# alanqrwang/nwhead

Measured on AMD Instinct MI355X. Metric: query-predictions/sec, higher is better.
Workload: dtype f32; 1 GPU; K3 predict('full'): B=256 queries/step vs bank N=50000 d=512 C=200, bank sharded 1-way, 26 query batches coalesced per launch; B=256, N_support=50000, d=512, C=200, parallelism=support-shard x1

## Files before the change

### nwhead_amd/csrc/fused.hip

```cpp
#include <mutex>
#include <utility>
#include <vector>
#include "fused_impl.h"
#include <cstring>

namespace nw {

#define NW_EXTERN_FUSED_KIND(K)                                                                          \
    extern template int launch_fused_kind<K>(const float*, const float*, const int64_t*, const float*,   \
                                             const float*,                                               \
                                             const float*, float*, float*, float*, float*, float*,       \
                                             float*, void*, size_t, int, int, int, int, hipStream_t);
NW_EXTERN_FUSED_KIND(NW_SCORE_EUCLIDEAN)
NW_EXTERN_FUSED_KIND(NW_SCORE_HYPERSPHERE)
NW_EXTERN_FUSED_KIND(NW_SCORE_COSINE)
NW_EXTERN_FUSED_KIND(NW_SCORE_DOT)
NW_EXTERN_FUSED_KIND(NW_SCORE_CLIP)
#undef NW_EXTERN_FUSED_KIND

namespace {
struct TileTimer {
    bool on = false;
    std::vector<std::pair<hipEvent_t, hipEvent_t>> ev;
    std::vector<std::pair<hipEvent_t, hipEvent_t>> pool;
    std::mutex mu;
} g_tt;
}

int tile_timer_start(hipStream_t st) {
    if (!g_tt.on) return -1;
    std::lock_guard<std::mutex> lk(g_tt.mu);
    std::pair<hipEvent_t, hipEvent_t> p;
    if (!g_tt.pool.empty()) {
        p = g_tt.pool.back();
        g_tt.pool.pop_back();
    } else if (hipEventCreate(&p.first) != hipSuccess || hipEventCreate(&p.second) != hipSuccess) {
        return -1;
    }
    (void)hipEventRecord(p.first, st);
    g_tt.ev.push_back(p);
    return (int)g_tt.ev.size() - 1;
}
void tile_timer_stop(int slot, hipStream_t st) {
    if (slot < 0) return;
    std::lock_guard<std::mutex> lk(g_tt.mu);
    if (slot < (int)g_tt.ev.size()) (void)hipEventRecord(g_tt.ev[slot].second, st);
}
int tile_timer_enable(bool on) {
    std::lock_guard<std::mutex> lk(g_tt.mu);
    g_tt.on = on;
    return NW_OK;
}
int tile_timer_read(double* total_us, int64_t* launches) {
    std::lock_guard<std::mutex> lk(g_tt.mu);
    double tot = 0;
    for (auto& p : g_tt.ev) {
        float ms = 0.f;
        if (hipEventSynchronize(p.second) != hipSuccess || hipEventElapsedTime(&ms, p.first, p.second) != hipSuccess)
            return NW_ERR_LAUNCH;
        tot += (double)ms * 1e3;
        g_tt.pool.push_back(p);
    }
    if (total_us) *total_us = tot;
    if (launches) *launches = (int64_t)g_tt.ev.size();
    g_tt.ev.clear();
    return NW_OK;
}

int persistent_variant() {
    const int x = knob(KNOB_PVAR);
    return (x >= 0 && x <= 2) ? x : -1;
}

int persistent_qgroup() {
    const int x = knob(KNOB_QG);
    return (x >= 1 && x <= 64) ? x : 8;
}

int device_cu_count() {
    static int n = [] {
        int dev = 0, v = 0;
        if (hipGetDevice(&dev) != hipSuccess) return 256;
        if (hipDeviceGetAttribute(&v, hipDeviceAttributeMultiprocessorCount, dev) != hipSuccess || v <= 0) return 256;
        return v;
    }();
    return n;
}
bool env_flag(const char* name) {
    static const struct { const char* n; int k; } map[] = {
        {"NW_MERGE_PER_QUERY", KNOB_MERGE_PER_QUERY}, {"NW_MERGE_NO_GLOBAL_TABLES", KNOB_MERGE_NO_GLOBAL_TABLES},
        {"NW_PERSISTENT_ANY_RS", KNOB_PERSISTENT_ANY_RS}, {"NW_NO_PERSISTENT", KNOB_NO_PERSISTENT}};
    for (const auto& m : map)
        if (!strcmp(m.n, name)) return knob(m.k) == 1;
    return false;
}

inline size_t al256(size_t x) { return (x + 255) & ~(size_t)255; }

size_t fused_layout(int64_t B, int64_t n_stiles, int BS, char* base, FusedWs* ws, int64_t C) {
    size_t off = 0;
    auto take = [&](size_t bytes) {
        char* p = base ? base + off : nullptr;
        off += al256(bytes);
        return p;
    };
    FusedWs w;
    w.m = reinterpret_cast<float*>(take((size_t)n_stiles * B * 4));
    w.den = reinterpret_cast<float*>(take((size_t)n_stiles * B * 4));
    w.nrun = reinterpret_cast<int*>(take((size_t)n_stiles * 4));
    w.lab = reinterpret_cast<int*>(take((size_t)n_stiles * BS * 4));
    w.num = reinterpret_cast<float*>(take((size_t)n_stiles * BS * B * 4));
    w.runid = reinterpret_cast<int*>(take(((size_t)n_stiles * BS + 64) * 4));
    w.bnd = reinterpret_cast<int*>(take((size_t)n_stiles * 2 * 4));
    w.ctab = reinterpret_cast<int*>(take((size_t)C * (3 + 4) * 4));
    if (ws) *ws = w;
    return off;
}

namespace {

constexpr int MTHREADS = 512, MENT = 4, MTPT = 16;
template <bool PARTIAL, int MQ, int TMODE>
__global__ __launch_bounds__(MTHREADS) void nw_merge_runs_kernel(
    const float* __restrict__ ws_m, const float* __restrict__ ws_den, const int* __restrict__ ws_nrun,
    const int* __restrict__ ws_lab, const float* __restrict__ ws_num, float* __restrict__ out,
    float* __restrict__ lse, float* __restrict__ m_out, float* __restrict__ den_out,
    float* __restrict__ num_out, int B, int C, int n_stiles, int BS, const int* __restrict__ ctab) {
    constexpr bool TABLES = TMODE != 0;
    constexpr bool LTAB = TMODE == 1;
    constexpr int ML = MTHREADS / MQ;
    constexpr int MNS = MQ + 1;
    constexpr int NW = MTHREADS / 64;
    constexpr float LN2 = 0.693147180559945309417f;
    static_assert(MQ <= 32 && (MQ & (MQ - 1)) == 0, "a wave holds whole groups of MQ queries");
    extern __shared__ __attribute__((aligned(16))) char smem[];
    float* red = reinterpret_cast<float*>(smem);
    float* Ms = red + 2 * NW * MQ;
    float* inv_s = Ms + MQ;
    int* lds_tab = reinterpret_cast<int*>(inv_s + MQ);
    int* cnt = TMODE == 2 ? const_cast<int*>(ctab) : lds_tab;
    int* tlo = cnt + C;
    int* thi = tlo + C;
    int* ent = thi + C;
    float* res = reinterpret_cast<float*>(lds_tab + (size_t)C * (3 + MENT));
    const int tid = threadIdx.x, bq = tid & (MQ - 1), sl = tid / MQ, wave = tid >> 6;
    const int b0 = blockIdx.x * MQ;
    const int b = min(b0 + bq, B - 1);

    const bool in_regs = n_stiles <= ML * MTPT;
    float mr[MTPT], dr[MTPT];
    float M = -INFINITY;
    if (in_regs) {
#pragma unroll
        for (int u = 0; u < MTPT; ++u) {
            const int t = sl + u * ML;
            const bool ok = t < n_stiles;
            mr[u] = ok ? ws_m[(size_t)t * B + b] : -INFINITY;
            dr[u] = ok ? ws_den[(size_t)t * B + b] : 0.f;
        }
    }
    int tnr = 0, tl3[3] = {-1, -1, -1};
    const bool one_pass_tables = LTAB && n_stiles <= MTHREADS;
    if (one_pass_tables && tid < n_stiles) {
        tnr = ws_nrun[tid];
        const int* lt = ws_lab + (size_t)tid * BS;
        tl3[0] = lt[0];
        tl3[1] = lt[1];
        tl3[2] = lt[2];
    }
    if (LTAB) {
        for (int c = tid; c < C; c += MTHREADS) {
            cnt[c] = 0;
            tlo[c] = 0x7fffffff;
            thi[c] = -1;
        }
    }
    if (in_regs) {
#pragma unroll
        for (int u = 0; u < MTPT; ++u) M = fmaxf(M, mr[u]);
    } else {
        for (int t = sl; t < n_stiles; t += ML) M = fmaxf(M, ws_m[(size_t)t * B + b]);
    }
#pragma unroll
    for (int o = 32; o >= MQ; o >>= 1) M = fmaxf(M, __shfl_xor(M, o));
    if ((tid & 63) < MQ) red[wave * MQ + bq] = M;
    __syncthreads();
    if (LTAB) {
        auto add_tile = [&](int t, int nr, const int (&l3)[3]) {
            const int* lt = ws_lab + (size_t)t * BS;
            for (int r = 0; r < nr; ++r) {
                const int y = r < 3 ? l3[r] : lt[r];
                if (y < 0) continue;
                atomicMin(&tlo[y], t);
                atomicMax(&thi[y], t);
                const int slot = atomicAdd(&cnt[y], 1);
                if (slot < MENT) ent[y * MENT + slot] = t * BS + r;
            }
        };
        if (one_pass_tables) {
            if (tid < n_stiles) add_tile(tid, tnr, tl3);
        } else {
            for (int t = tid; t < n_stiles; t += MTHREADS) {
                const int* lt = ws_lab + (size_t)t * BS;
                const int l3[3] = {lt[0], lt[1], lt[2]};
                add_tile(t, ws_nrun[t], l3);
            }
        }
    }
    M = red[bq];
#pragma unroll
    for (int k = 1; k < NW; ++k) M = fmaxf(M, red[k * MQ + bq]);
    float den = 0.f;
    if (in_regs) {
#pragma unroll
        for (int u = 0; u < MTPT; ++u) den += dr[u] * __builtin_amdgcn_exp2f(mr[u] - M);
    } else {
        for (int t = sl; t < n_stiles; t += ML)
            den += ws_den[(size_t)t * B + b] * __builtin_amdgcn_exp2f(ws_m[(size_t)t * B + b] - M);
    }
#pragma unroll
    for (int o = 32; o >= MQ; o >>= 1) den += __shfl_xor(den, o);
    if ((tid & 63) < MQ) red[NW * MQ + wave * MQ + bq] = den;
    if (sl == 0) Ms[bq] = M;
    __syncthreads();
    if (LTAB) {
        for (int c = tid; c < C; c += MTHREADS) {
            const int n = cnt[c];
            if (n > 1 && n <= MENT) {
                int e[MENT];
#pragma unroll
                for (int k = 0; k < MENT; ++k) e[k] = k < n ? ent[c * MENT + k] : 0x7fffffff;
#pragma unroll
                for (int i = 1; i < MENT; ++i)
#pragma unroll
                    for (int j = MENT - 1; j >= i; --j)
                        if (e[j] < e[j - 1]) { const int x = e[j]; e[j] = e[j - 1]; e[j - 1] = x; }
#pragma unroll
                for (int k = 0; k < MENT; ++k)
                    if (k < n) ent[c * MENT + k] = e[k];
            }
        }
    }
    den = red[NW * MQ + bq];
#pragma unroll
    for (int k = 1; k < NW; ++k) den += red[NW * MQ + k * MQ + bq];
    if (sl == 0) inv_s[bq] = 1.f / den;
    const int nq = min(MQ, B - b0);
    if (sl == 0 && bq < nq) {
        if (PARTIAL) {
            m_out[b] = M * LN2;
            den_out[b] = den;
        } else if (lse) {
            lse[b] = M * LN2 + logf(den);
        }
    }
    __syncthreads();
    int P = 1;
    while (P < 64 && 2 * P * C * MQ <= MTHREADS) P <<= 1;
    for (int xx = tid; xx < C * MQ * P; xx += MTHREADS) {
        const int x = xx / P, sub = xx - x * P;
        const int c = x / MQ, q = x - c * MQ;
        const int bb = min(b0 + q, B - 1);
        const float Mq = Ms[q];
        float acc = 0.f;
        const int n = TABLES ? cnt[c] : MENT + 1;
        if (n <= MENT) {
            int e[MENT];
            float v[MENT], mt[MENT];
#pragma unroll
            for (int k = 0; k < MENT; ++k) e[k] = ent[c * MENT + (k < n ? k : 0)];
#pragma unroll
            for (int k = 0; k < MENT; ++k) {
                if (k < n) {
                    v[k] = ws_num[(size_t)e[k] * B + bb];
                    mt[k] = ws_m[(size_t)(e[k] / BS) * B + bb];
                }
            }
#pragma unroll
            for (int k = 0; k < MENT; ++k)
                if (k < n) acc += v[k] * __builtin_amdgcn_exp2f(mt[k] - Mq);
        } else {
            const int t0 = TABLES ? tlo[c] : 0, t1 = TABLES ? thi[c] : n_stiles - 1;
            for (int t = t0 + sub; t <= t1; t += P) {
                const int nr = ws_nrun[t];
                const float f = __builtin_amdgcn_exp2f(ws_m[(size_t)t * B + bb] - Mq);
                const int* lt = ws_lab + (size_t)t * BS;
                for (int r = 0; r < nr; ++r)
                    if (lt[r] == c) acc += ws_num[((size_t)t * BS + r) * B + bb] * f;
            }
        }
        if (P > 1) {
            if (n <= MENT && sub != 0) acc = 0.f;
            for (int o = P >> 1; o > 0; o >>= 1) acc += __shfl_xor(acc, o);
            if (sub != 0) continue;
        }
        if (LTAB && MQ > 1) {
            res[c * MNS + q] = acc;
        } else if (q < nq) {
            if (PARTIAL) num_out[(size_t)bb * C + c] = acc;
            else out[(size_t)bb * C + c] = logf(acc * inv_s[q] + NW_LOG_EPS);
        }
    }
    if (!LTAB || MQ == 1) return;
    __syncthreads();
    for (int x = tid; x < nq * C; x += MTHREADS) {
        const int qq = x / C, c = x - qq * C;
        if (PARTIAL) num_out[(size_t)(b0 + qq) * C + c] = res[c * MNS + qq];
        else out[(size_t)(b0 + qq) * C + c] = logf(res[c * MNS + qq] * inv_s[qq] + NW_LOG_EPS);
    }
}

__global__ __launch_bounds__(1024) void nw_class_tables_kernel(const int* __restrict__ ws_nrun, const int* __restrict__ ws_lab,
                                                                int n_stiles, int BS, int C, int* __restrict__ ctab) {
    int* cnt = ctab;
    int* tlo = cnt + C;
    int* thi = tlo + C;
    int* ent = thi + C;
    const int tid = threadIdx.x;
    for (int c = tid; c < C; c += 1024) {
        cnt[c] = 0;
        tlo[c] = 0x7fffffff;
        thi[c] = -1;
    }
    __threadfence();
    __syncthreads();
    for (int t = tid; t < n_stiles; t += 1024) {
        const int nr = ws_nrun[t];
        const int* lt = ws_lab + (size_t)t * BS;
        for (int r = 0; r < nr; ++r) {
            const int y = lt[r];
            if (y < 0) continue;
            atomicMin(&tlo[y], t);
            atomicMax(&thi[y], t);
            const int slot = atomicAdd(&cnt[y], 1);
            if (slot < MENT) ent[y * MENT + slot] = t * BS + r;
        }
    }
    __threadfence();
    __syncthreads();
    for (int c = tid; c < C; c += 1024) {
        const int n = cnt[c];
        if (n > 1 && n <= MENT) {
            int e[MENT];
#pragma unroll
            for (int k = 0; k < MENT; ++k) e[k] = k < n ? ent[c * MENT + k] : 0x7fffffff;
#pragma unroll
            for (int i = 1; i < MENT; ++i)
#pragma unroll
                for (int j = MENT - 1; j >= i; --j)
                    if (e[j] < e[j - 1]) { const int x = e[j]; e[j] = e[j - 1]; e[j - 1] = x; }
#pragma unroll
            for (int k = 0; k < MENT; ++k)
                if (k < n) ent[c * MENT + k] = e[k];
        }
    }
}

__global__ __launch_bounds__(64) void nw_run_tables_kernel(const int64_t* __restrict__ sy, int N, int C, int BS,
                                                           int* __restrict__ runid, int* __restrict__ nrun,
                                                           int* __restrict__ lab_out, int* __restrict__ bnd) {
    const int st = blockIdx.x, lane = threadIdx.x, s0 = st * BS;
    if (lane < 2) bnd[2 * st + lane] = BS;
    __syncthreads();
    int lab[3], flag[3];
#pragma unroll
    for (int u = 0; u < 3; ++u) {
        const int t = 3 * lane + u, j = s0 + t;
        int64_t y = -1;
        if (t < BS && j < N) y = sy[j];
        lab[u] = ((uint64_t)y < (uint64_t)C) ? (int)y : -1;
    }
    const int prev_last = __shfl_up(lab[2], 1);
    flag[0] = (lane == 0) || (lab[0] != prev_last);
    flag[1] = lab[1] != lab[0];
// ... 201 lines not shown
```

### nwhead_amd/csrc/fused_impl.h

```cpp
#pragma once
#include <type_traits>
#include "tile_core.h"
#include "tile_dma.h"
#include "tile_f16.h"

namespace nw {

constexpr int RUN_CAP = 192;

struct FusedWs {
    float* m;
    float* den;
    int* nrun;
    int* lab;
    float* num;
    int* runid;
    int* bnd;
    int* ctab;
};
size_t fused_layout(int64_t B, int64_t n_stiles, int BS, char* base, FusedWs* ws, int64_t C = 0);
int launch_run_tables(const FusedWs& ws, const int64_t* sy, int N, int C, int n_stiles, int BS, hipStream_t st);
bool bank_tables_take(const int64_t* sy, int N, int C, int n_stiles, int BS, FusedWs* ws);
int launch_merge_runs(const FusedWs& ws, float* out, float* lse, float* m, float* den, float* num,
                      int B, int C, int n_stiles, int BS, hipStream_t st);
// ... 82 lines not shown
        float Cq, Bq;
        SF::query(qn, qsc, scale, Cq, Bq);
#pragma unroll
        for (int r = 0; r < RS; ++r) {
            float4 n2 = make_float4(0.f, 0.f, 0.f, 0.f), s4 = make_float4(1.f, 1.f, 1.f, 1.f);
            if (NEED_NORM) n2 = *reinterpret_cast<const float4*>(sn2 + 16 * r + 4 * g);
            if (mode_is_f16(MODE)) s4 = *reinterpret_cast<const float4*>(ssc + 16 * r + 4 * g);
            const float nn[4] = {n2.x, n2.y, n2.z, n2.w}, ss[4] = {s4.x, s4.y, s4.z, s4.w};
#pragma unroll
            for (int e = 0; e < 4; ++e) {
                float K, Base;
                SF::support(nn[e], ss[e], K, Base);
                sc[r][e] = SF::finish(__builtin_fmaf(acc[r][e], K * Cq, Base + Bq));
            }
        }
        if (partial_tile) {
#pragma unroll
            for (int r = 0; r < RS; ++r)
#pragma unroll
                for (int e = 0; e < 4; ++e)
                    if (s0 + 16 * r + 4 * g + e >= N) sc[r][e] = -INFINITY;
        }
#pragma unroll
        for (int r = 0; r < RS; ++r) mloc = fmaxf(mloc, fmaxf(fmaxf(sc[r][0], sc[r][1]), fmaxf(sc[r][2], sc[r][3])));
        if (WRITE_SCORES && b < B) {
            float* orow = scores + (size_t)b * N;
            const bool vec_ok = (N & 3) == 0;
#pragma unroll
            for (int r = 0; r < RS; ++r) {
                const int j = s0 + 16 * r + 4 * g;
                if (j >= N) continue;
                if (vec_ok) {
                    *reinterpret_cast<float4*>(orow + j) =
                        make_float4(sc[r][0] * LN2, sc[r][1] * LN2, sc[r][2] * LN2, sc[r][3] * LN2);
                } else {
#pragma unroll
                    for (int e = 0; e < 4; ++e)
                        if (j + e < N) orow[j + e] = sc[r][e] * LN2;
                }
            }
        }
        mloc = group4_max(mloc);
    }
    NW_FSTAMP(3);

    if (consumer) {
        float dloc = 0.f;
#pragma unroll
        for (int r = 0; r < RS; ++r)
#pragma unroll
            for (int e = 0; e < 4; ++e) sc[r][e] = __builtin_amdgcn_exp2f(sc[r][e] - mloc);
        const int nrun = nrun_s[0];
        if (nrun <= 3) {
            float S0[2] = {0.f, 0.f}, S1[2] = {0.f, 0.f}, S2[2] = {0.f, 0.f};
            if (nrun == 1) {
#pragma unroll
                for (int r = 0; r < RS; ++r) S0[r & 1] += (sc[r][0] + sc[r][1]) + (sc[r][2] + sc[r][3]);
            } else if (nrun == 2) {
                const float L1 = (float)(nrun_s[1] - 4 * g), M1 = 1.f - L1;
#pragma unroll
                for (int r = 0; r < RS; ++r)
#pragma unroll
                    for (int e = 0; e < 4; ++e) {
                        const float c = (float)(16 * r + e), ev = sc[r][e];
                        S0[e & 1] = __builtin_fmaf(__builtin_amdgcn_fmed3f(L1 - c, 0.f, 1.f), ev, S0[e & 1]);
                        S1[e & 1] = __builtin_fmaf(__builtin_amdgcn_fmed3f(c + M1, 0.f, 1.f), ev, S1[e & 1]);
                    }
            } else {
                const float L1 = (float)(nrun_s[1] - 4 * g);
                const float M2 = 1.f - (float)(nrun_s[2] - 4 * g);
#pragma unroll
                for (int r = 0; r < RS; ++r)
#pragma unroll
                    for (int e = 0; e < 4; ++e) {
                        const float c = (float)(16 * r + e), ev = sc[r][e];
                        const float w1 = __builtin_amdgcn_fmed3f(L1 - c, 0.f, 1.f);
                        const float u2 = __builtin_amdgcn_fmed3f(c + M2, 0.f, 1.f);
                        S0[e & 1] = __builtin_fmaf(w1, ev, S0[e & 1]);
                        S2[e & 1] = __builtin_fmaf(u2, ev, S2[e & 1]);
                        S1[e & 1] = __builtin_fmaf((1.f - w1) - u2, ev, S1[e & 1]);
                    }
            }
            const float s0v = group4_sum(S0[0] + S0[1]);
            float s1v = 0.f, s2v = 0.f;
            if (nrun >= 2) s1v = group4_sum(S1[0] + S1[1]);
            if (nrun == 3) s2v = group4_sum(S2[0] + S2[1]);
            dloc = (s0v + s1v) + s2v;
            if (g == 0 && b < B) {
                ws_num[((size_t)st * BS) * B + b] = s0v;
                if (nrun >= 2) ws_num[((size_t)st * BS + 1) * B + b] = s1v;
                if (nrun == 3) ws_num[((size_t)st * BS + 2) * B + b] = s2v;
            }
        } else {
            float dl[4] = {0.f, 0.f, 0.f, 0.f};
#pragma unroll
            for (int r = 0; r < RS; ++r) dl[r & 3] += (sc[r][0] + sc[r][1]) + (sc[r][2] + sc[r][3]);
            dloc = group4_sum((dl[0] + dl[1]) + (dl[2] + dl[3]));
            for (int run_base = 0; run_base < nrun; run_base += 16) {
                f32x4 P0 = {0.f, 0.f, 0.f, 0.f}, P1 = P0, P2 = P0, P3 = P0;
                const int want = run_base + i;
#pragma unroll
                for (int r = 0; r < RS; ++r) {
                    const int4 rid = *reinterpret_cast<const int4*>(runid + 16 * r + 4 * g);
                    P0 = __builtin_amdgcn_mfma_f32_16x16x4f32(rid.x == want ? 1.f : 0.f, sc[r][0], P0, 0, 0, 0);
                    P1 = __builtin_amdgcn_mfma_f32_16x16x4f32(rid.y == want ? 1.f : 0.f, sc[r][1], P1, 0, 0, 0);
                    P2 = __builtin_amdgcn_mfma_f32_16x16x4f32(rid.z == want ? 1.f : 0.f, sc[r][2], P2, 0, 0, 0);
                    P3 = __builtin_amdgcn_mfma_f32_16x16x4f32(rid.w == want ? 1.f : 0.f, sc[r][3], P3, 0, 0, 0);
                }
                const f32x4 P = (P0 + P1) + (P2 + P3);
                if (b < B) {
#pragma unroll
                    for (int j = 0; j < 4; ++j) {
                        const int run = run_base + 4 * g + j;
                        if (run < nrun) ws_num[((size_t)st * BS + run) * B + b] = P[j];
                    }
                }
            }
        }
        NW_FSTAMP(4);
        if (g == 0 && b < B) {
            ws_m[(size_t)st * B + b] = mloc;
            ws_den[(size_t)st * B + b] = dloc;
        }
    }
    NW_FSTAMP(5);
    if (qt == 0) {
        const int nrun = *nrun_s;
        if (tid == 0) ws_nrun[st] = nrun;
        for (int x = tid; x < nrun; x += TILE_THREADS) ws_lab[(size_t)st * BS + x] = runlab[x];
    }
}


template <int RS, int KIND, bool WRITE_SCORES, int MODE>
__global__ __launch_bounds__(TILE_THREADS, (RS <= 5 ? 4 : 2)) void nw_fused_kernel(
    const float* __restrict__ q, const float* __restrict__ s, const int64_t* __restrict__ sy,
    const float* __restrict__ s_norm2, const float* __restrict__ s_scale, const float* __restrict__ q_norm2,
    const float* __restrict__ q_scale, const float* __restrict__ logit_scale,
    float* __restrict__ scores, float* __restrict__ ws_m,
    float* __restrict__ ws_den, int* __restrict__ ws_nrun, int* __restrict__ ws_lab,
    float* __restrict__ ws_num, int B, int N, int d, int C, int n_stiles, int n_qtiles) {
    using Cfg = TileCfg<RS>;
    constexpr int BS = Cfg::BS;
    constexpr bool NEED_NORM = (KIND != NW_SCORE_DOT);
    extern __shared__ __attribute__((aligned(16))) char smem[];
    float* qn2 = reinterpret_cast<float*>(smem);
    float* qsc_s = qn2 + 64;
    float* sn2 = qsc_s + 64;
    float* ssc = sn2 + RUN_CAP;
    int* runid = reinterpret_cast<int*>(ssc + RUN_CAP);
    int* runlab = runid + RUN_CAP;
    int* nrun_s = runlab + RUN_CAP;
    constexpr int HDR = (128 + 4 * RUN_CAP + 4) * 4;
    static_assert(HDR % 16 == 0, "stage buffers must stay 16-byte aligned");
    float4* stage = reinterpret_cast<float4*>(smem + HDR);

    int qt, st;
    if (!decode_block(n_stiles, n_qtiles, qt, st)) return;
    const int q0 = qt * BQ, s0 = st * BS;
    const int tid = threadIdx.x, wave = tid >> 6, lane = tid & 63;
    const int i = lane & 15, g = lane >> 4;
    NW_FSTAMP(0);

    if ((MODE == MODE_DMA_SN || mode_is_f16(MODE)) && NEED_NORM) {
        for (int t = tid; t < BS; t += TILE_THREADS) sn2[t] = s_norm2[min(s0 + t, N - 1)];
    }
    if (mode_is_f16(MODE)) {
        for (int t = tid; t < BS; t += TILE_THREADS) ssc[t] = s_scale[min(s0 + t, N - 1)];
    }
    if (MODE == MODE_F16) {
        if (NEED_NORM)
            for (int t = tid; t < BQ; t += TILE_THREADS) qn2[t] = q_norm2[min(q0 + t, B - 1)];
        for (int t = tid; t < BQ; t += TILE_THREADS) qsc_s[t] = q_scale[min(q0 + t, B - 1)];
    }
    if (wave == 0) {
        int lab[3];
        load_tile_labels<BS>(sy, s0, N, C, lane, lab);
        run_scan_wave<BS>(lab, lane, runid, runlab, nrun_s);
    }

    NW_FSTAMP(1);
    const int nk = (d + BK - 1) / BK;
    const int rot = st % nk;
    f32x4 acc[RS];
    if (mode_is_f16(MODE)) {
        tile_dots_f16x2<RS, MODE == MODE_F16Q>(q, s, B, N, d, q0, s0, stage, acc, rot, qn2, qsc_s);
        __syncthreads();
    } else if (MODE == MODE_REG) {
        tile_dots<RS, NEED_NORM>(q, s, B, N, d, q0, s0, stage, qn2, sn2, acc, rot);
    } else {
        tile_dots_dma<RS, NEED_NORM, NEED_NORM && MODE == MODE_DMA>(q, s, B, N, d, q0, s0, stage, qn2, sn2, acc, rot);
    }
    if (MODE != MODE_DMA_SN && !mode_is_f16(MODE) && NEED_NORM && s_norm2 != nullptr) {
        for (int t = tid; t < BS; t += TILE_THREADS) sn2[t] = s_norm2[min(s0 + t, N - 1)];
        __syncthreads();
    }

    NW_FSTAMP(2);
    fused_epilogue<RS, KIND, WRITE_SCORES, MODE>(acc, qn2, sn2, ssc, runid, runlab, nrun_s, qsc_s, logit_scale,
                                                 scores, ws_m, ws_den, ws_nrun, ws_lab, ws_num, B, N, q0, s0, qt, st);
    NW_FSTAMP(6);
}


constexpr size_t FUSED_HDR = (128 + 4 * RUN_CAP + 4) * 4;

template <int RS, int KIND>
int launch_f16p(const float* q, const float* s, const int64_t* sy, const float* s_norm2, const float* s_scale,
                const float* q_norm2, const float* q_scale, const float* ls, const FusedWs& ws, int B, int N,
                int d, int C, int n_stiles, int n_qtiles, hipStream_t st);

template <int RS, int KIND>
int launch_fused_rs(const float* q, const float* s, const int64_t* sy, const float* s_norm2,
                    const float* s_scale,
                    const float* ls, float* out, float* scores, float* lse, float* m, float* den,
                    float* num, void* workspace, size_t workspace_bytes, int B, int N, int d, int C,
                    hipStream_t st) {
    const float *q_norm2 = nullptr, *q_scale = nullptr;
    constexpr int BS = 16 * RS;
    const int n_stiles = (N + BS - 1) / BS;
    const int n_qtiles = (B + BQ - 1) / BQ;
    FusedWs ws;
    const size_t need = fused_layout(B, n_stiles, BS, static_cast<char*>(workspace), &ws, C);
    if (!workspace || workspace_bytes < need) return NW_ERR_WORKSPACE;
    const int grid = padded_grid(n_stiles, n_qtiles);
    const bool dma = (d % BK) == 0 && (uint64_t)(BQ + BS) * 2 * d * 4 < 0xffffffffull;
    if (!dma && (RS & 1)) return NW_ERR_UNSUPPORTED;
    const size_t lds_reg = FUSED_HDR + TileCfg<RS>::STAGE_BYTES, lds_dma = FUSED_HDR + DmaCfg<RS>::STAGE_BYTES;
#define NW_LAUNCH(WS_, MODE_, LDS_)                                                                      \
    hipLaunchKernelGGL((nw_fused_kernel<RS, KIND, WS_, MODE_>), dim3(grid), dim3(TILE_THREADS), LDS_, st, \
                       q, s, sy, s_norm2, s_scale, q_norm2, q_scale, ls, scores, ws.m, ws.den, ws.nrun, ws.lab, \
                       ws.num, B, N, d, C,                                                                  \
                       n_stiles, n_qtiles)
    const bool persistent = s_scale && !scores && RS > 5 && (RS == 8 || env_flag("NW_PERSISTENT_ANY_RS")) &&
                            grid >= 4 * device_cu_count() && d >= 3 * BK && !env_flag("NW_NO_PERSISTENT");
    if (persistent) {
        if (!bank_tables_take(sy, N, C, n_stiles, 16 * RS, &ws)) {
            const int rc = launch_run_tables(ws, sy, N, C, n_stiles, 16 * RS, st);
            if (rc != NW_OK) return rc;
        }
    }
    if (s_scale) {
        if (!dma || !s_norm2) return NW_ERR_INVALID_ARG;
        const int force_split = knob(KNOB_SPLIT_QUERIES) == KNOB_UNSET ? -1 : knob(KNOB_SPLIT_QUERIES);
        const bool raw_ok = force_split == 0 || (force_split < 0 && 2 * grid <= 3 * device_cu_count());
        if (persistent || !raw_ok) {
            float *qr, *qsc, *qn;
            const int rc = split_queries_into_workspace(q, workspace, workspace_bytes, B, N, d, C, &qr, &qsc, &qn, st);
            if (rc != NW_OK) return rc;
            q = qr;
            q_scale = qsc;
            q_norm2 = qn;
        }
    }
    const int timer_slot = tile_timer_start(st);
    if (s_scale) {
        if (!q_scale) {
            if (scores) NW_LAUNCH(true, MODE_F16Q, lds_dma); else NW_LAUNCH(false, MODE_F16Q, lds_dma);
        } else if (scores) {
            NW_LAUNCH(true, MODE_F16, lds_dma);
        } else if (persistent) {
            const int rc = launch_f16p<RS, KIND>(q, s, sy, s_norm2, s_scale, q_norm2, q_scale, ls, ws, B, N, d, C,
                                                 n_stiles, n_qtiles, st);
            if (rc != NW_OK) return rc;
        } else {
            NW_LAUNCH(false, MODE_F16, lds_dma);
        }
    } else if (dma && s_norm2 && KIND != NW_SCORE_DOT) {
        if (scores) NW_LAUNCH(true, MODE_DMA_SN, lds_dma); else NW_LAUNCH(false, MODE_DMA_SN, lds_dma);
    } else if (dma) {
        if (scores) NW_LAUNCH(true, MODE_DMA, lds_dma); else NW_LAUNCH(false, MODE_DMA, lds_dma);
    } else {
        if (scores) NW_LAUNCH(true, MODE_REG, lds_reg); else NW_LAUNCH(false, MODE_REG, lds_reg);
    }
#undef NW_LAUNCH
    tile_timer_stop(timer_slot, st);
    NW_CHECK_LAUNCH();
    return launch_merge_runs(ws, out, lse, m, den, num, B, C, n_stiles, BS, st);
}

}

template <int KIND>
int launch_fused_kind(const float* q, const float* s, const int64_t* sy, const float* s_norm2,
                      const float* s_scale,
                      const float* ls, float* out, float* scores, float* lse, float* m, float* den,
                      float* num, void* workspace, size_t wsb, int B, int N, int d, int C, hipStream_t st) {
#define NW_RS_CASE(R) \
    case R: return launch_fused_rs<R, KIND>(q, s, sy, s_norm2, s_scale, ls, out, scores, lse, m, den, num, workspace, wsb, B, N, d, C, st)
    switch (pick_rs(B, N, d, s_scale != nullptr)) {
        NW_RS_CASE(2);
        NW_RS_CASE(4);
        NW_RS_CASE(5);
        NW_RS_CASE(6);
        NW_RS_CASE(8);
        NW_RS_CASE(10);
        default: return launch_fused_rs<12, KIND>(q, s, sy, s_norm2, s_scale, ls, out, scores, lse, m, den, num, workspace, wsb, B, N, d, C, st);
    }
#undef NW_RS_CASE
}

}
#include "fused_f16p.h"
#ifdef NW_WITH_P8
#include "fused_f16p8.h"
#endif
namespace nw {
namespace {
template <int RS, int KIND>
int launch_f16p(const float* q, const float* s, const int64_t* sy, const float* s_norm2, const float* s_scale,
                const float* q_norm2, const float* q_scale, const float* ls, const FusedWs& ws, int B, int N,
                int d, int C, int n_stiles, int n_qtiles, hipStream_t st) {
    if constexpr (RS > 5) {
        (void)sy; (void)C;
        int cus = device_cu_count() & ~7;
        const int wg_cap = fwd_opts().persistent_wgs & ~7;
        if (wg_cap >= 8 && wg_cap < cus) cus = wg_cap;
        int variant = persistent_variant();
        if (variant < 0) variant = ((B + 127) / 128 * 128 <= 1.15 * ((B + 63) / 64 * 64)) ? 2 : 1;
        (void)n_qtiles;
#ifdef NW_WITH_P8
        if constexpr (RS == 8) {
            if (variant == 3) {
                static const bool attr = hipFuncSetAttribute(reinterpret_cast<const void*>(nw_fused_f16p8_kernel<KIND>),
                                                             hipFuncAttributeMaxDynamicSharedMemorySize, (int)P8::LDS_BYTES) == hipSuccess;
                (void)attr;
                int qgrp = persistent_qgroup() / 2;
                if (qgrp < 1) qgrp = 1;
                hipLaunchKernelGGL((nw_fused_f16p8_kernel<KIND>), dim3(cus), dim3(TILE_THREADS), P8::LDS_BYTES, st, q, s, s_norm2,
                                   s_scale, q_norm2, q_scale, ls, ws.runid, ws.nrun, ws.bnd, ws.m, ws.den, ws.num, B, N, d, n_stiles,
                                   (B + P8::BQP - 1) / P8::BQP, qgrp);
                NW_CHECK_LAUNCH();
                return NW_OK;
            }
        }
#endif
        if (variant > 2) variant = 2;
#define NW_LAUNCH_P(TWO_, QB_, GRID_, NBUF_)                                                                      \
    do {                                                                                                          \
        using PC_ = PCfg<RS, QB_>;                                                                                \
        const size_t lds_ = PC_::HDR_BYTES + (size_t)(NBUF_) * PC_::TILE_F4 * 16;                                 \
        hipLaunchKernelGGL((nw_fused_f16p_kernel<RS, KIND, TWO_, QB_>), dim3(GRID_), dim3(TILE_THREADS), lds_, st, \
                           q, s, s_norm2, s_scale, q_norm2, q_scale, ls, ws.runid, ws.nrun, ws.bnd, ws.m, ws.den, ws.num,  \
                           B, N, d, n_stiles, (B + 64 * (QB_) - 1) / (64 * (QB_)), persistent_qgroup());          \
    } while (0)
        constexpr size_t lds_q2 = PCfg<RS, 2>::HDR_BYTES + (size_t)4 * PCfg<RS, 2>::TILE_F4 * 16;
        constexpr size_t lds_two = PCfg<RS, 1>::HDR_BYTES + (size_t)3 * PCfg<RS, 1>::TILE_F4 * 16;
        if (variant == 2 && lds_q2 <= 160 * 1024) {
            NW_LAUNCH_P(false, 2, cus, 4);
        } else if (variant == 1 && lds_two <= 80 * 1024) {
            NW_LAUNCH_P(true, 1, 2 * cus, 3);
        } else {
            NW_LAUNCH_P(false, 1, cus, 4);
        }
#undef NW_LAUNCH_P
        NW_CHECK_LAUNCH();
    }
    return NW_OK;
}
}

#define NW_INSTANTIATE_FUSED_KIND(K)                                                                   \
    template int launch_fused_kind<K>(const float*, const float*, const int64_t*, const float*,        \
                                      const float*,                                                    \
                                      const float*, float*, float*, float*, float*, float*, float*,    \
                                      void*, size_t, int, int, int, int, hipStream_t);

}
```

Baseline: 6.660 million query-predictions/s.

## Add warp-specialized 12-wave persistent kernel with dedicated DMA waves as default

Adds a new persistent fused kernel in which 8 compute waves run the f16 MFMA tiles over 256 queries and 4 loader waves stream query/support tiles and headers into a 3-stage LDS ring through global_load_lds. The launcher selects it by default when RS==8 and B pads cleanly to 256 rows. The aim is to take global-to-LDS transfer issue off the compute waves and to raise query reuse per support tile. In exchange, LDS use per workgroup grows, occupancy drops, and wave scheduling becomes more complex.

Result: faster. 7.529 million query-predictions/s, median of 6 (+13.1%).

```diff
diff --git a/nwhead_amd/csrc/fused.hip b/nwhead_amd/csrc/fused.hip
--- a/nwhead_amd/csrc/fused.hip
+++ b/nwhead_amd/csrc/fused.hip
@@ -69,7 +69,7 @@
 
 int persistent_variant() {
     const int x = knob(KNOB_PVAR);
-    return (x >= 0 && x <= 2) ? x : -1;
+    return (x >= 0 && x <= 3) ? x : -1;
 }
 
 int persistent_qgroup() {
diff --git a/nwhead_amd/csrc/fused_f16p12.h b/nwhead_amd/csrc/fused_f16p12.h
--- /dev/null
+++ b/nwhead_amd/csrc/fused_f16p12.h
@@ -0,0 +1,466 @@
+#pragma once
+#include "fused_f16p.h"
+
+namespace nw {
+namespace {
+
+struct P12 {
+    static constexpr int RS = 8, QB = 2, NCW = 8, NLW = 4;
+    static constexpr int THREADS = 64 * (NCW + NLW);
+    static constexpr int BS = 16 * RS;
+    static constexpr int BQP = 16 * QB * NCW;
+    static constexpr int ROWS = BQP + BS;
+    static constexpr int TILE_F4 = ROWS * ROW_F4;
+    static constexpr int STAGE_BYTES = TILE_F4 * 16;
+    static constexpr int NB = 3;
+    static constexpr int AHEAD = NB - 1;
+    static constexpr int NT = ROWS / 8;
+    static constexpr int NI = NT / NLW;
+    static constexpr int NQI = BQP / 8 / NLW;
+    static constexpr int N64 = BS / 64;
+    static constexpr int NH = BS;
+    static constexpr int HDR_F = 3 * NH + 2 * BQP;
+    static constexpr int NP = 3 * N64 + 2 * (BQP / 64);
+    static constexpr int HPW = (NP + NLW - 1) / NLW;
+    static constexpr int NHB = 3;
+    static constexpr size_t HDR_BYTES = (size_t)NHB * HDR_F * 4;
+    static constexpr size_t LDS_BYTES = HDR_BYTES + (size_t)NB * STAGE_BYTES;
+    static_assert(NT % NLW == 0 && (BQP / 8) % NLW == 0, "even split of the pieces");
+    static_assert(HDR_BYTES % 16 == 0 && LDS_BYTES <= 160 * 1024, "LDS of one CU");
+    static_assert(NI + HPW < 64, "vmcnt is a 6-bit field");
+};
+
+template <int KIND>
+__device__ __forceinline__ void epilogue_p12(f32x4 (&acc)[P12::QB][P12::RS], const float* hdr, int nrun, int2 bnd,
+                                             float scale, float* __restrict__ ws_m,
+                                             float* __restrict__ ws_den, float* __restrict__ ws_num, int B, int N,
+                                             int q0, int s0, int st, int wave, int lane
+#ifdef NW_DIAG_FUSED
+                                             , unsigned long long (&diag_)[8], unsigned long long& last_
+#endif
+                                             ) {
+    using P = P12;
+    constexpr int RS = P::RS, QB = P::QB, BS = P::BS;
+    constexpr bool NEED_NORM = (KIND != NW_SCORE_DOT);
+    typedef float f32x2 __attribute__((ext_vector_type(2)));
+    const float* sn2 = hdr;
+    const float* ssc = hdr + P::NH;
+    const int* runid = reinterpret_cast<const int*>(hdr + 2 * P::NH);
+    const float* qn2 = hdr + 3 * P::NH;
+    const float* qsc_s = qn2 + P::BQP;
+    const int i = lane & 15, g = lane >> 4;
+    using SF = ScoreFactors<KIND>;
+    float Cq[QB], Bq[QB];
+#pragma unroll
+    for (int j = 0; j < QB; ++j) {
+        const int qrow = 16 * (QB * wave + j) + i;
+        SF::query(NEED_NORM ? qn2[qrow] : 0.f, qsc_s[qrow], scale, Cq[j], Bq[j]);
+    }
+    NW_PSTAMP(1);
+    float sc[QB][RS][4];
+#pragma unroll
+    for (int r = 0; r < RS; ++r) {
+        const float4 n4 = NEED_NORM ? *reinterpret_cast<const float4*>(sn2 + 16 * r + 4 * g) : make_float4(0.f, 0.f, 0.f, 0.f);
+        const float4 s4 = *reinterpret_cast<const float4*>(ssc + 16 * r + 4 * g);
+        float4 K4, B4;
+        SF::support(n4.x, s4.x, K4.x, B4.x);
+        SF::support(n4.y, s4.y, K4.y, B4.y);
+        SF::support(n4.z, s4.z, K4.z, B4.z);
+        SF::support(n4.w, s4.w, K4.w, B4.w);
+        float4 B4r = B4;
+        asm volatile("" : "+v"(B4r.x), "+v"(B4r.y), "+v"(B4r.z), "+v"(B4r.w));
+#pragma unroll
+        for (int j = 0; j < QB; ++j) {
+            const f32x2 cq = {Cq[j], Cq[j]}, bq = {Bq[j], Bq[j]};
+            const float4 Bj = (j == 0) ? B4 : B4r;
+            const f32x2 d01 = __builtin_elementwise_fma(f32x2{acc[j][r][0], acc[j][r][1]}, f32x2{K4.x, K4.y} * cq,
+                                                        f32x2{Bj.x, Bj.y} + bq);
+            const f32x2 d23 = __builtin_elementwise_fma(f32x2{acc[j][r][2], acc[j][r][3]}, f32x2{K4.z, K4.w} * cq,
+                                                        f32x2{Bj.z, Bj.w} + bq);
+            sc[j][r][0] = SF::finish_abs(d01.x);
+            sc[j][r][1] = SF::finish_abs(d01.y);
+            sc[j][r][2] = SF::finish_abs(d23.x);
+            sc[j][r][3] = SF::finish_abs(d23.y);
+            asm volatile("" : "+v"(sc[j][r][0]), "+v"(sc[j][r][1]), "+v"(sc[j][r][2]), "+v"(sc[j][r][3]));
+        }
+        __builtin_amdgcn_sched_barrier(0);
+    }
+    NW_PSTAMP(2);
+#pragma unroll
+    for (int j = 0; j < QB; ++j) {
+        const int qrow = 16 * (QB * wave + j) + i;
+        const int b = q0 + qrow;
+        float (&sj)[RS][4] = sc[j];
+        constexpr float WORST = SF::DIST ? INFINITY : -INFINITY;
+        if (s0 + BS > N) {
+            const int lim = N - s0 - 4 * g;
+#pragma unroll
+            for (int r = 0; r < RS; ++r)
+#pragma unroll
+                for (int e = 0; e < 4; ++e)
+                    if (16 * r + e >= lim) sj[r][e] = WORST;
+        }
+        auto best = [](float a, float b) { return SF::DIST ? fminf(a, b) : fmaxf(a, b); };
+        float mx[4] = {WORST, WORST, WORST, WORST};
+#pragma unroll
+        for (int r = 0; r < RS; ++r) mx[r & 3] = best(mx[r & 3], best(best(sj[r][0], sj[r][1]), best(sj[r][2], sj[r][3])));
+        float ext = best(best(mx[0], mx[1]), best(mx[2], mx[3]));
+        ext = SF::DIST ? group4_min(ext) : group4_max(ext);
+        const float mloc = SF::DIST ? -ext : ext;
+#pragma unroll
+        for (int r = 0; r < RS; ++r)
+#pragma unroll
+            for (int e = 0; e < 4; ++e)
+                sj[r][e] = __builtin_amdgcn_exp2f(SF::DIST ? ext - sj[r][e] : sj[r][e] - ext);
+        NW_PSTAMP(3);
+        float dloc;
+        auto red4 = [](float x) { return group4_sum(x); };
+        if (nrun <= 3) {
+            float S0[2] = {0.f, 0.f}, S1[2] = {0.f, 0.f}, S2[2] = {0.f, 0.f};
+            if (nrun == 1) {
+#pragma unroll
+                for (int r = 0; r < RS; ++r) {
+                    S0[r & 1] += (sj[r][0] + sj[r][1]) + (sj[r][2] + sj[r][3]);
+                }
+            } else {
+                const int b1 = bnd.x, b2 = (nrun == 3) ? bnd.y : BS;
+                const float L1 = (float)(b1 - 4 * g);
+                const float M2 = 1.f - (float)(b2 - 4 * g);
+#pragma unroll
+                for (int r = 0; r < RS; ++r) {
+                    const int lo = 16 * r, hi = 16 * r + 16;
+                    const bool in0 = hi <= b1, in2 = lo >= b2, in1 = lo >= b1 && hi <= b2;
+                    const float quad = (sj[r][0] + sj[r][1]) + (sj[r][2] + sj[r][3]);
+                    S0[r & 1] = __builtin_fmaf(in0 ? 1.f : 0.f, quad, S0[r & 1]);
+                    S1[r & 1] = __builtin_fmaf(in1 ? 1.f : 0.f, quad, S1[r & 1]);
+                    S2[r & 1] = __builtin_fmaf(in2 ? 1.f : 0.f, quad, S2[r & 1]);
+                    if (!(in0 || in1 || in2)) {
+#pragma unroll
+                        for (int e = 0; e < 4; ++e) {
+                            const float c = (float)(16 * r + e), ev = sj[r][e];
+                            const float w1 = __builtin_amdgcn_fmed3f(L1 - c, 0.f, 1.f);
+                            const float u2 = __builtin_amdgcn_fmed3f(c + M2, 0.f, 1.f);
+                            S0[e & 1] = __builtin_fmaf(w1, ev, S0[e & 1]);
+                            S2[e & 1] = __builtin_fmaf(u2, ev, S2[e & 1]);
+                            S1[e & 1] = __builtin_fmaf((1.f - w1) - u2, ev, S1[e & 1]);
+                        }
+                    }
+                }
+            }
+            const float s0v = red4(S0[0] + S0[1]);
+            float s1v = 0.f, s2v = 0.f;
+            if (nrun >= 2) s1v = red4(S1[0] + S1[1]);
+            if (nrun == 3) s2v = red4(S2[0] + S2[1]);
+            dloc = (s0v + s1v) + s2v;
+            if (g == 0 && b < B) {
+                ws_num[((size_t)st * BS) * B + b] = s0v;
+                if (nrun >= 2) ws_num[((size_t)st * BS + 1) * B + b] = s1v;
+                if (nrun == 3) ws_num[((size_t)st * BS + 2) * B + b] = s2v;
+            }
+        } else {
+            float dl[4] = {0.f, 0.f, 0.f, 0.f};
+#pragma unroll
+            for (int r = 0; r < RS; ++r) dl[r & 3] += (sj[r][0] + sj[r][1]) + (sj[r][2] + sj[r][3]);
+            dloc = red4((dl[0] + dl[1]) + (dl[2] + dl[3]));
+            for (int run_base = 0; run_base < nrun; run_base += 16) {
+                f32x4 Pm = {0.f, 0.f, 0.f, 0.f};
+                const int want = run_base + i;
+#pragma unroll
+                for (int r = 0; r < RS; ++r) {
+                    const int4 rid = *reinterpret_cast<const int4*>(runid + 16 * r + 4 * g);
+                    Pm = __builtin_amdgcn_mfma_f32_16x16x4f32(rid.x == want ? 1.f : 0.f, sj[r][0], Pm, 0, 0, 0);
+                    Pm = __builtin_amdgcn_mfma_f32_16x16x4f32(rid.y == want ? 1.f : 0.f, sj[r][1], Pm, 0, 0, 0);
+                    Pm = __builtin_amdgcn_mfma_f32_16x16x4f32(rid.z == want ? 1.f : 0.f, sj[r][2], Pm, 0, 0, 0);
+                    Pm = __builtin_amdgcn_mfma_f32_16x16x4f32(rid.w == want ? 1.f : 0.f, sj[r][3], Pm, 0, 0, 0);
+                }
+                if (b < B) {
+#pragma unroll
+                    for (int jj = 0; jj < 4; ++jj) {
+                        const int run = run_base + 4 * g + jj;
+                        if (run < nrun) ws_num[((size_t)st * BS + run) * B + b] = Pm[jj];
+                    }
+                }
+            }
+        }
+        NW_PSTAMP(4);
+        if (g == 0 && b < B) {
+            ws_m[(size_t)st * B + b] = mloc;
+            ws_den[(size_t)st * B + b] = dloc;
+        }
+        NW_PSTAMP(5);
+    }
+}
+
+template <int KIND>
+__global__ __launch_bounds__(P12::THREADS, 3) void nw_fused_f16p_kernel_w12(
+    const float* __restrict__ q, const float* __restrict__ s, const float* __restrict__ s_norm2,
+    const float* __restrict__ s_scale, const float* __restrict__ q_norm2, const float* __restrict__ q_scale,
+    const float* __restrict__ logit_scale, const int* __restrict__ ws_runid, const int* __restrict__ ws_nrun,
+    const int* __restrict__ ws_bnd, float* __restrict__ ws_m, float* __restrict__ ws_den, float* __restrict__ ws_num, int B,
+    int N, int d, int n_stiles, int n_qtiles, int qg) {
+    using P = P12;
+    constexpr int RS = P::RS, QB = P::QB, BS = P::BS, BQP = P::BQP, NI = P::NI, NB = P::NB, NLW = P::NLW;
+    extern __shared__ __attribute__((aligned(16))) char smem[];
+    float* hdr0 = reinterpret_cast<float*>(smem);
+    float4* stage = reinterpret_cast<float4*>(smem + P::HDR_BYTES);
+
+    const int tid = threadIdx.x, lane = tid & 63;
+    const int wave = __builtin_amdgcn_readfirstlane(tid >> 6);
+    const int nk = d / BK;
+    const int xcd = blockIdx.x & 7, cu = blockIdx.x >> 3, n_cu = gridDim.x >> 3;
+    const int ns_x = n_stiles >> 3;
+    const int n_full = ns_x * n_qtiles;
+    const int rem = n_stiles & 7;
+    const int nq_x = (n_qtiles - xcd + 7) >> 3;
+    const int n_local = n_full + rem * nq_x;
+    const int grp_tiles = qg * ns_x;
+    auto decode = [&](int L, int& qt, int& st) {
+        if (L >= n_full) {
+            const int r = L - n_full, j = r / nq_x;
+            st = 8 * ns_x + j;
+            qt = xcd + 8 * (r - j * nq_x);
+            return;
+        }
+        const int gi_ = L / grp_tiles, r = L - gi_ * grp_tiles;
+        const int g_ = min(qg, n_qtiles - gi_ * qg);
+        const int stl = r / g_;
+        qt = gi_ * qg + (r - stl * g_);
+        st = stl * 8 + xcd;
+    };
+
+    if (wave >= P::NCW) {
+        const int lw = wave - P::NCW;
+        unsigned voff[NI];
+        int iT = cu, ikt = 0, irot = 0, ipar = 0;
+        int iq0 = 0, is0 = 0, ist = 0;
+        int gs = 0;
+        auto set_tile = [&](int T) {
+            int qt, st;
+            decode(T, qt, st);
+            iq0 = qt * BQP;
+            is0 = st * BS;
+            ist = st;
+            irot = st % nk;
+#pragma unroll
+            for (int m = 0; m < NI; ++m) {
+                const int R = 8 * (lw + NLW * m) + (lane >> 3);
+                const int lslot = (lane & 7) ^ ((R >> 1) & 7);
+                const int rel = (m < P::NQI) ? min(iq0 + R, B - 1) - iq0 : min(is0 + R - BQP, N - 1) - is0;
+                voff[m] = ((unsigned)rel * (unsigned)d + lslot * 4) * 4u;
+            }
+        };
+        auto dma4 = [&](const void* src, float* dst) {
+            __builtin_amdgcn_global_load_lds((const __attribute__((address_space(1))) void*)src,
+                                             (__attribute__((address_space(3))) void*)dst, 4, 0, 0);
+        };
+        auto issue_header = [&]() {
+            float* h = hdr0 + ipar * P::HDR_F;
+#pragma unroll
+            for (int k = 0; k < P::HPW; ++k) {
+                const int pc = min(lw + NLW * k, P::NP - 1);
+                if (pc < 3 * P::N64) {
+                    const int arr = pc / P::N64, c = pc - arr * P::N64;
+                    const int row = is0 + 64 * c + lane;
+                    float* dst = h + arr * P::NH + 64 * c;
+                    if (arr == 0) dma4(s_norm2 + min(row, N - 1), dst);
+                    else if (arr == 1) dma4(s_scale + min(row, N - 1), dst);
+                    else dma4(ws_runid + (size_t)ist * BS + 64 * c + lane, dst);
+                } else {
+                    const int qp = pc - 3 * P::N64, arr = qp / (BQP / 64), c = qp - arr * (BQP / 64);
+                    const int row = min(iq0 + 64 * c + lane, B - 1);
+                    dma4((arr == 0 ? q_norm2 : q_scale) + row, h + 3 * P::NH + arr * BQP + 64 * c);
+                }
+            }
+        };
+        bool young_hdr = false;
+        auto issue_next = [&]() {
+            if (iT >= n_local) return false;
+            int kc = ikt + irot;
+            if (kc >= nk) kc -= nk;
+            float4* buf = stage + gs * P::TILE_F4;
+            const char* qb = reinterpret_cast<const char*>(q + (size_t)iq0 * d) + (size_t)kc * BK * 4;
+            const char* sb = reinterpret_cast<const char*>(s + (size_t)is0 * d) + (size_t)kc * BK * 4;
+#ifndef NW_ABL_NODMA
+#pragma unroll
+            for (int m = 0; m < NI; ++m) {
+                const char* g = ((m < P::NQI) ? qb : sb) + voff[m];
+                __builtin_amdgcn_global_load_lds((const __attribute__((address_space(1))) void*)g,
+                                                 (__attribute__((address_space(3))) void*)(buf + 64 * (lw + NLW * m)), 16, 0, 0);
+            }
+#else
+            (void)qb; (void)sb; (void)buf;
+#endif
+            young_hdr = (ikt == 0);
+            if (young_hdr) issue_header();
+            gs = (gs + 1 == NB) ? 0 : gs + 1;
+            if (++ikt == nk) {
+                ikt = 0;
+                ipar = (ipar + 1 == P::NHB) ? 0 : ipar + 1;
+                iT += n_cu;
+                if (iT < n_local) set_tile(iT);
+            }
+            return true;
+        };
+        auto wait_landed = [&](bool issued) {
+#ifdef NW_ABL_NODMA
+            if (!issued) wait_vmcnt<0>();
+            else if (young_hdr) wait_vmcnt<P::HPW>();
+            else wait_vmcnt<0>();
+#else
+            if (!issued) wait_vmcnt<0>();
+            else if (young_hdr) wait_vmcnt<NI + P::HPW>();
+            else wait_vmcnt<NI>();
+#endif
+        };
+        if (iT < n_local) set_tile(iT);
+        bool more = true;
+#pragma unroll
+        for (int k0 = 0; k0 < P::AHEAD; ++k0) more = issue_next();
+        wait_landed(more);
+        tile_barrier();
+        for (int T = cu; T < n_local; T += n_cu) {
+            for (int kt = 0; kt < nk; ++kt) {
+                more = issue_next();
+                wait_landed(more);
+                tile_barrier();
+            }
+        }
+    } else {
+        const int i = lane & 15, g = lane >> 4;
+        const int rsw = (i >> 1) & 7;
+        const int sh = g ^ rsw, sl = (4 + g) ^ rsw;
+        const int qoff = (16 * QB * wave + i) * ROW_F4, soff = (BQP + i) * ROW_F4;
+        struct QF { float4 bh[QB], bl[QB]; };
+        struct SW { float4 al[2], ah[2]; };
+        constexpr int NW_ = RS / 2;
+        auto rd_q = [&](QF& f, const float4* S) {
+#pragma unroll
+            for (int j = 0; j < QB; ++j) {
+                f.bh[j] = S[qoff + 16 * j * ROW_F4 + sh];
+                f.bl[j] = S[qoff + 16 * j * ROW_F4 + sl];
+            }
+        };
+        auto rd_w = [&](SW& w, const float4* S, int p) {
+#pragma unroll
+            for (int x = 0; x < 2; ++x) {
+                w.al[x] = S[soff + 16 * (2 * p + x) * ROW_F4 + sl];
+                w.ah[x] = S[soff + 16 * (2 * p + x) * ROW_F4 + sh];
+            }
+        };
+        auto mm = [](const float4& a, const float4& b, f32x4 c) {
+            return __builtin_amdgcn_mfma_f32_16x16x32_f16(__builtin_bit_cast(half8, a), __builtin_bit_cast(half8, b), c, 0, 0, 0);
+        };
+        auto pin = []() { __builtin_amdgcn_sched_barrier(0); };
+        f32x4 acc[QB][RS];
+        auto mm_w = [&](const SW& w, const QF& f, int p) {
+#pragma unroll
+            for (int x = 0; x < 2; ++x)
+#pragma unroll
+                for (int j = 0; j < QB; ++j) acc[j][2 * p + x] = mm(w.al[x], f.bh[j], acc[j][2 * p + x]);
+#pragma unroll
+            for (int x = 0; x < 2; ++x)
+#pragma unroll
+                for (int j = 0; j < QB; ++j) acc[j][2 * p + x] = mm(w.ah[x], f.bl[j], acc[j][2 * p + x]);
+#pragma unroll
+            for (int x = 0; x < 2; ++x)
+#pragma unroll
+                for (int j = 0; j < QB; ++j) acc[j][2 * p + x] = mm(w.ah[x], f.bh[j], acc[j][2 * p + x]);
+            __builtin_amdgcn_sched_barrier(0);
+        };
+        SW wa, wb;
+        auto run_stage = [&](const QF& fp, QF& fc, int slot, auto first) {
+            constexpr bool FIRST = decltype(first)::value;
+#ifdef NW_ABL_NORD
+            constexpr bool RD = FIRST;
+#else
+            constexpr bool RD = true;
+#endif
+            const float4* S = stage + slot * P::TILE_F4;
+            if (RD) { rd_q(fc, S); rd_w(wa, S, 0); }
+            pin();
+            if (!FIRST) mm_w(wb, fp, NW_ - 1);
+#pragma unroll
+            for (int p = 0; p + 1 < NW_; ++p) {
+                if (RD) rd_w((p & 1) ? wa : wb, S, p + 1);
+                pin();
+                mm_w((p & 1) ? wb : wa, fc, p);
+            }
+            static_assert(NW_ % 2 == 0, "the last pair of a stage sits in wb");
+            tile_barrier();
+        };
+        using Yes = std::integral_constant<bool, true>;
+        using No = std::integral_constant<bool, false>;
+
+        float scale = 1.f;
+        if (KIND == NW_SCORE_CLIP)
+            scale = __builtin_bit_cast(float, __builtin_amdgcn_readfirstlane(__builtin_bit_cast(int, expf(*logit_scale))));
+        tile_barrier();
+        int gi = 0;
+        int par = 0;
+        auto next_slot = [&]() {
+            const int b = gi;
+            gi = (gi + 1 == NB) ? 0 : gi + 1;
+            return b;
+        };
+#ifdef NW_DIAG_FUSED
+        unsigned long long diag_[8] = {0, 0, 0, 0, 0, 0, 0, 0}, last_ = __builtin_amdgcn_s_memtime();
+        const unsigned long long first_ = last_, first_rt_ = __builtin_amdgcn_s_memrealtime();
+#endif
+        for (int T = cu; T < n_local; T += n_cu) {
+            int qt, st;
+            decode(T, qt, st);
+            const int q0 = qt * BQP, s0 = st * BS;
+            const int nrun = ws_nrun[st];
+            const int2 bnd = *reinterpret_cast<const int2*>(ws_bnd + 2 * (size_t)st);
+#pragma unroll
+            for (int j = 0; j < QB; ++j)
+#pragma unroll
+                for (int r = 0; r < RS; ++r) acc[j][r] = f32x4{0.f, 0.f, 0.f, 0.f};
+            QF f0, f1;
+#ifdef NW_ABL_NORD
+            rd_q(f1, stage + gi * P::TILE_F4);
+#endif
+            run_stage(f1, f0, next_slot(), Yes{});
+            int kt = 1;
+            for (; kt + 1 < nk; kt += 2) {
+                run_stage(f0, f1, next_slot(), No{});
+                run_stage(f1, f0, next_slot(), No{});
+            }
+            if (kt < nk) {
+                run_stage(f0, f1, next_slot(), No{});
+                mm_w(wb, f1, NW_ - 1);
+            } else {
+                mm_w(wb, f0, NW_ - 1);
+            }
+            NW_PSTAMP(0);
+#ifndef NW_ABL_NOEPI
+            epilogue_p12<KIND>(acc, hdr0 + par * P::HDR_F, nrun, bnd, scale, ws_m, ws_den, ws_num, B, N, q0, s0, st, wave,
+                               lane
+#ifdef NW_DIAG_FUSED
+                               , diag_, last_
+#endif
+                               );
+#else
+            {
+                f32x4 sum_ = {0.f, 0.f, 0.f, 0.f};
+                for (int j = 0; j < QB; ++j)
+                    for (int r = 0; r < RS; ++r) sum_ += acc[j][r];
+                if (sum_[0] + sum_[1] + sum_[2] + sum_[3] == 12345.678f) ws_m[tid] = sum_[0] + nrun + bnd.x;
+            }
+#endif
+            par = (par + 1 == P::NHB) ? 0 : par + 1;
+            NW_PSTAMP(6);
+        }
+#ifdef NW_DIAG_FUSED
+        if (tid == 0 && blockIdx.x < 1024) {
+            for (int k = 0; k < 7; ++k) nw_diag_p[8 * blockIdx.x + k] = diag_[k];
+            nw_diag_p[8 * blockIdx.x + 7] = last_ - first_;
+            nw_diag_rt[2 * blockIdx.x] = first_rt_;
+            nw_diag_rt[2 * blockIdx.x + 1] = __builtin_amdgcn_s_memrealtime();
+        }
+#endif
+    }
+}
+
+}
+}
diff --git a/nwhead_amd/csrc/fused_impl.h b/nwhead_amd/csrc/fused_impl.h
--- a/nwhead_amd/csrc/fused_impl.h
+++ b/nwhead_amd/csrc/fused_impl.h
@@ -408,9 +408,7 @@
 
 }
 #include "fused_f16p.h"
-#ifdef NW_WITH_P8
-#include "fused_f16p8.h"
-#endif
+#include "fused_f16p12.h"
 namespace nw {
 namespace {
 template <int RS, int KIND>
@@ -423,24 +421,25 @@
         const int wg_cap = fwd_opts().persistent_wgs & ~7;
         if (wg_cap >= 8 && wg_cap < cus) cus = wg_cap;
         int variant = persistent_variant();
-        if (variant < 0) variant = ((B + 127) / 128 * 128 <= 1.15 * ((B + 63) / 64 * 64)) ? 2 : 1;
+        if (variant < 0) {
+            const double rows64 = 1.15 * ((B + 63) / 64 * 64);
+            variant = (RS == 8 && (B + 255) / 256 * 256 <= rows64) ? 3 : ((B + 127) / 128 * 128 <= rows64) ? 2 : 1;
+        }
         (void)n_qtiles;
-#ifdef NW_WITH_P8
         if constexpr (RS == 8) {
             if (variant == 3) {
-                static const bool attr = hipFuncSetAttribute(reinterpret_cast<const void*>(nw_fused_f16p8_kernel<KIND>),
-                                                             hipFuncAttributeMaxDynamicSharedMemorySize, (int)P8::LDS_BYTES) == hipSuccess;
+                static const bool attr = hipFuncSetAttribute(reinterpret_cast<const void*>(nw_fused_f16p_kernel_w12<KIND>),
+                                                             hipFuncAttributeMaxDynamicSharedMemorySize, (int)P12::LDS_BYTES) == hipSuccess;
                 (void)attr;
                 int qgrp = persistent_qgroup() / 2;
                 if (qgrp < 1) qgrp = 1;
-                hipLaunchKernelGGL((nw_fused_f16p8_kernel<KIND>), dim3(cus), dim3(TILE_THREADS), P8::LDS_BYTES, st, q, s, s_norm2,
-                                   s_scale, q_norm2, q_scale, ls, ws.runid, ws.nrun, ws.bnd, ws.m, ws.den, ws.num, B, N, d, n_stiles,
-                                   (B + P8::BQP - 1) / P8::BQP, qgrp);
+                hipLaunchKernelGGL((nw_fused_f16p_kernel_w12<KIND>), dim3(cus), dim3(P12::THREADS), P12::LDS_BYTES, st, q, s,
+                                   s_norm2, s_scale, q_norm2, q_scale, ls, ws.runid, ws.nrun, ws.bnd, ws.m, ws.den, ws.num, B, N, d,
+                                   n_stiles, (B + P12::BQP - 1) / P12::BQP, qgrp);
                 NW_CHECK_LAUNCH();
                 return NW_OK;
             }
         }
-#endif
         if (variant > 2) variant = 2;
 #define NW_LAUNCH_P(TWO_, QB_, GRID_, NBUF_)                                                                      \
     do {                                                                                                          \
```
